# simongoricar/diploma_thesis-distributed_rendering_of_cgi_using_a_render_cluster

Measured on AMD Instinct MI355X. Metric: job frames/sec at 1/2/4/8 MI355X (04_very-simple); Mrays/s per GPU, higher is better.
Workload: dtype f32

## Files before the change

diploma_thesis-distributed_rendering_of_cgi_using_a_render_cluster_amd/csrc/paths.hpp:

```cpp
#pragma once

#include <hip/hip_runtime.h>

#include <algorithm>
#include <map>
#include <type_traits>
#include <utility>

#include "device.hpp"

namespace rr {

struct SceneArgs {
    const BvhNode* nodes;
    const QNode6* qnodes;
    const TriPack* tris;
    const float* mats;
    const float* lights;
    const float* filter;
    const float* mat_lut;
    int n_nodes, n_tris, n_mats, n_lights;
    int n_qnodes;
};

// ... 217 lines not shown
                const float3 wl = scl3(tl, rl);
                float3 b1, b2;
                make_onb(wl, b1, b2);
                float dx, dy;
                float u1, u2;
                rng2(key, dim0 + 1u, u1, u2);
                concentric_disk(u1, u2, dx, dy);
                dx = dx * radius;
                dy = dy * radius;
                const float3 sp = madd3(madd3(lp, b1, dx), b2, dy);
                const float3 ts = sub3(sp, P);
                const float ds2 = dot3(ts, ts);
                float id;
                sqrt_rcp_any(ds2, dist, id);
                wi = scl3(ts, id);
                const float cl = fabsf(dot3(wl, wi));
                Li = scl3(I, cl * id * id);
            } else {
                float id;
                sqrt_rcp_any(dl2, dist, id);
                wi = scl3(tl, id);
                Li = scl3(I, 1.0f / dl2);
            }
        } else {
            wi = mk3(-lt[4], -lt[5], -lt[6]);
            dist = kFltMax;
            Li = mk3(lt[8], lt[9], lt[10]);
        }
        const float cosN = dot3(N, wi);
        if (cosN > 0.0f) {
            float pdf;
            const float3 f = bsdf_eval_v(m, lut, vw, N, wo, wi, pdf);
            const float k = (float)fc.n_lights;
            float3 c = mk3(T.x * f.x * k * Li.x, T.y * f.y * k * Li.y, T.z * f.z * k * Li.z);
            if (bounce > 0) c = clamp_contrib(c, fc.clamp_indirect);
            if (max3f(c) > 0.0f) {
                out.shadow = true;
                if constexpr (Shadow::kInline) {
                    if (esc || !trace_shadow(Po, wi, dist)) add_to(L, c);
                } else {
                    out.so = Po;
                    out.sd = wi;
                    out.sdist = dist;
                    out.sc = c;
                }
            }
        }
    }
    float3 wi, f;
    float pdf;
    bool glossy;
    float u_b1, u_b2;
    rng2(key, dim0 + 4u, u_b1, u_b2);
    bool sampled;
    if constexpr (std::is_same<View, LdsView>::value) {
        const lds_f4w* fr = v.onb + kOnbF4 * h.idx + (flip ? 2 : 0);
        const float4 tb = lds_ld4(fr), bb = lds_ld4(fr + 1);
        sampled = bsdf_sample_onb(m, lut, vw, N, xyz(tb), mk3(tb.w, bb.x, bb.y), wo, u_lobe, u_b1, u_b2, wi, f, pdf,
                                  glossy);
    } else {
        sampled = bsdf_sample(m, lut, vw, N, wo, u_lobe, u_b1, u_b2, wi, f, pdf, glossy);
    }
    if (!sampled) return;
    const float k = 1.0f / pdf;
    T = mk3(T.x * f.x * k, T.y * f.y * k, T.z * f.z * k);
    if (!(max3f(T) > 0.0f)) return;
    if (bounce >= kRrStartBounce) {
        const float q = fminf(max3f(T), 1.0f);
        if (rng(key, dim0 + 6u) >= q) return;
        const float iq = 1.0f / q;
        T = mk3(T.x * iq, T.y * iq, T.z * iq);
    }
    out.cont = true;
    if constexpr (Cont::kInline) {
        on_cont(Po, wi, T, lob + (glossy ? kGlossyOne : 1u), esc, L);
        return;
    }
    out.o = Po;
    out.d = wi;
    out.T = T;
    out.lob = lob + (glossy ? kGlossyOne : 1u);
}

constexpr int kWavesPerBlock = kBlock / 64;
constexpr int kMaxBlocksPerCu = 8;

__device__ __forceinline__ void flush_counts(unsigned long long* __restrict__ tc, int slot, uint32_t nv,
                                             uint32_t nt) {
    unsigned long long a = nv, b = nt;
    for (int off = 32; off > 0; off >>= 1) {
        a += __shfl_xor(a, off);
        b += __shfl_xor(b, off);
    }
    if ((threadIdx.x & 63) == 0) {
        atomicAdd(&tc[slot], a);
        atomicAdd(&tc[slot + 1], b);
    }
}

RR_D void set_miss(Hit& h, float tmax) {
    h.t = tmax;
    h.u = h.v = 0.0f;
    h.idx = -1;
    h.orig = -1;
}

RR_D uchar4 tonemap(const FrameConsts& fc, float4 acc, const float* __restrict__ srgb) {
    float c[3] = {acc.x * fc.inv_spp * fc.exposure_scale, acc.y * fc.inv_spp * fc.exposure_scale,
                  acc.z * fc.inv_spp * fc.exposure_scale};
    uint8_t q[3];
    for (int k = 0; k < 3; ++k) {
        float v = fminf(fmaxf(c[k], 0.0f), 1.0f);
        if (fc.view_transform == 0) v = srgb_oetf(v, srgb, kSrgbN);
        q[k] = quantize8(v);
    }
    return make_uchar4(q[0], q[1], q[2], 255);
}

template <typename K>
int resident_grid(K kernel, size_t dyn_lds = 0, int block = kBlock) {
    int per_cu = 0;
    if (hipOccupancyMaxActiveBlocksPerMultiprocessor(&per_cu, kernel, block, dyn_lds) != hipSuccess || per_cu <= 0)
        per_cu = std::max(1, 1024 / block);
    return device_cu_count() * std::min(per_cu, kMaxBlocksPerCu * kBlock / block);
}
template <typename K>
int grid_for(K kernel, size_t dyn_lds, int block = kBlock) {
    static std::map<std::pair<const void*, size_t>, int> cache;
    const auto key = std::make_pair(reinterpret_cast<const void*>(kernel), dyn_lds);
    auto it = cache.find(key);
    if (it != cache.end()) return it->second;
    return cache[key] = resident_grid(kernel, dyn_lds, block);
}
inline int clamp_grid(long work, int resident, int block = kBlock) {
    const long g = (work + block - 1) / block;
    return (int)std::max<long>(1, std::min<long>(g, resident));
}

}
}
```

diploma_thesis-distributed_rendering_of_cgi_using_a_render_cluster_amd/csrc/rr_api.cpp:

```cpp
#include <hip/hip_runtime.h>

#include <cerrno>
#include <chrono>
#include <cmath>
#include <cstdlib>
#include <cstring>
#include <memory>
#include <string>
#include <unordered_set>
#include <vector>

#include "deflate.hpp"
#include "device.hpp"
#include "image_io.hpp"
#include "rr.h"
#include "scene.hpp"
#include "view.hpp"

using namespace rr;

static_assert(kMatLutIntervals == kMatLutN && kMatLutFloatsPerMat == kMatLutStride && kMatLutPsOffset == kMatLutPs,
              "scene.hpp material-table layout must match rr_device.h");

namespace {
// ... 1485 lines not shown
                    if (children) {
                        const uint32_t eb = (uint32_t)f2i(q.org.w);
                        for (int k = 0; k < kQWidth; ++k) {
                            const uint32_t lox = k < 4 ? (q.a.z >> (8 * k)) & 255u : (q.c.x >> (8 * (k - 4))) & 255u;
                            const uint32_t hix = k < 4 ? (q.b.y >> (8 * k)) & 255u : (q.c.y >> (16 + 8 * (k - 4))) & 255u;
                            const bool unused = lox == 255u && hix == 0u && !((eb >> (24 + k)) & 1u);
                            children[kQWidth * (size_t)i + k] = unused ? 0x7fffffff : q6_ref(q, k);
                        }
                    }
                    if (nodes16) std::memcpy(nodes16 + 16 * (size_t)i, &q, sizeof(QNode6));
                }
            }
            if (tri_orig) {
                std::vector<TriPack> tp((size_t)n);
                RR_HIP(hipMemcpyAsync(tp.data(), d.tris.ptr, (size_t)n * sizeof(TriPack), hipMemcpyDeviceToHost, st));
                RR_HIP(hipStreamSynchronize(st));
                for (int i = 0; i < n; ++i) tri_orig[i] = f2i(tp[(size_t)i].p0.w);
            }
        }
        return RR_OK;
    });
}

int rr_debug_trace(rr_ctx* c, rr_scene* s, int32_t frame, int32_t bvh_width, int32_t n, const float* rays,
                   float* hits, int32_t* prims, uint8_t* occluded) {
    if (!c || !s || n < 0 || (n > 0 && !rays)) return fail(RR_EINVAL, "bad arguments");
    if (bvh_width < 0 || bvh_width == 1 || bvh_width > 7)
        return fail(RR_EINVAL, "hierarchy must be 0 (frame's), 2 (LBVH), 3 (PLOC), 4 (6-wide), 5 (6-wide, packets) "
                               "6 (6-wide, one LDS stack entry) or 7 (6-wide, beam packets)");
    return guarded([&] {
        if (!idle(c)) return fail(RR_EBUSY, "submitted frames are pending");
        FrameSetup fs = setup_frame(s->desc, frame, nullptr);
        set_device(c);
        PinnedBuf staging;
        const int hier = bvh_width >= 5 ? kHierQWide : (bvh_width ? bvh_width : frame_hier_of(s, fs));
        prepare_frame(c, s, s->build, c->home, c->stream, fs, staging, hier);
        const int width = bvh_width >= 5 ? bvh_width : (hier == kHierQWide ? 4 : 2);
        hipStream_t st = c->stream;
        DevBuf<float4> dr, dh;
        DevBuf<int32_t> dp;
        DevBuf<uint8_t> dq;
        const size_t m = n > 0 ? (size_t)n : 1;
        dr.ensure(2 * m);
        dh.ensure(m);
        dp.ensure(m);
        dq.ensure(m);
        if (n > 0) RR_HIP(hipMemcpyAsync(dr.ptr, rays, (size_t)n * 8 * sizeof(float), hipMemcpyHostToDevice, st));
        trace_batch_device(s->mesh, s->build, c->paths, c->home, n, dr.ptr, dh.ptr, dp.ptr, dq.ptr, st, width);
        std::vector<float4> h(m);
        if (n > 0) {
            RR_HIP(hipMemcpyAsync(h.data(), dh.ptr, n * sizeof(float4), hipMemcpyDeviceToHost, st));
            if (prims) RR_HIP(hipMemcpyAsync(prims, dp.ptr, n * sizeof(int32_t), hipMemcpyDeviceToHost, st));
            if (occluded) RR_HIP(hipMemcpyAsync(occluded, dq.ptr, n, hipMemcpyDeviceToHost, st));
        }
        RR_HIP(hipStreamSynchronize(st));
        if (hits)
            for (int i = 0; i < n; ++i) {
                hits[4 * i] = h[i].x;
                hits[4 * i + 1] = h[i].y;
                hits[4 * i + 2] = h[i].z;
                hits[4 * i + 3] = 0.0f;
            }
        dr.release(); dh.release(); dp.release(); dq.release();
        return RR_OK;
    });
}

int rr_debug_tile_costs(rr_ctx* c, int32_t capacity, uint32_t* costs, int32_t* order, int32_t* n_tiles,
                        uint64_t* unit_log, int32_t unit_capacity) {
    if (!c || capacity < 0 || !n_tiles || (capacity > 0 && (!costs || !order)) || unit_capacity < 0 ||
        (unit_capacity > 0 && !unit_log))
        return fail(RR_EINVAL, "bad arguments");
    return guarded([&] {
        if (!idle(c)) return fail(RR_EBUSY, "submitted frames are pending");
        *n_tiles = 0;
        const FrameSlot* sl = c->last_enqueued;
        if (!sl || !sl->tiles) return RR_OK;
        set_device(c);
        const DevFrame& f = sl->dev;
        const size_t n = std::min(f.tile_cost.cap, f.tile_order.cap);
        *n_tiles = (int32_t)n;
        const size_t m = std::min<size_t>(n, (size_t)capacity);
        if (m > 0) {
            RR_HIP(hipMemcpy(costs, f.tile_cost.ptr, m * sizeof(uint32_t), hipMemcpyDeviceToHost));
            RR_HIP(hipMemcpy(order, f.tile_order.ptr, m * sizeof(int32_t), hipMemcpyDeviceToHost));
        }
        const size_t nu = std::min<size_t>((size_t)unit_capacity, kUnitLog);
        if (nu > 0) {
            std::memset(unit_log, 0, 2 * nu * sizeof(uint64_t));
            if (f.unit_logged && f.trav_counts.cap >= (size_t)(kTravWords + 2 * kUnitLog))
                RR_HIP(hipMemcpy(unit_log, f.trav_counts.ptr + kTravWords, 2 * nu * sizeof(uint64_t),
                                 hipMemcpyDeviceToHost));
        }
        return RR_OK;
    });
}

int rr_debug_fastmath_check(rr_ctx* c, uint32_t lo, uint64_t n, uint64_t* counts5) {
    if (!c || !counts5 || n > (1ull << 32) - lo) return fail(RR_EINVAL, "bad arguments");
    return guarded([&] {
        if (!idle(c)) return fail(RR_EBUSY, "submitted frames are pending");
        set_device(c);
        hipStream_t st = c->stream;
        DevBuf<unsigned long long> d;
        d.ensure(5);
        fastmath_check_device(lo, n, d.ptr, st);
        RR_HIP(hipMemcpyAsync(counts5, d.ptr, 5 * sizeof(uint64_t), hipMemcpyDeviceToHost, st));
        RR_HIP(hipStreamSynchronize(st));
        d.release();
        return RR_OK;
    });
}

int rr_debug_bsdf_sample(rr_ctx* c, const float* mat12, const float* n3, const float* wo3, int32_t n,
                         const float* u, float* wi3, float* f3, float* pdf, int32_t* ok) {
    if (!c || !mat12 || !n3 || !wo3 || n < 0 || (n > 0 && (!u || !wi3 || !f3 || !pdf || !ok)))
        return fail(RR_EINVAL, "bad arguments");
    return guarded([&] {
        if (!idle(c)) return fail(RR_EBUSY, "submitted frames are pending");
        set_device(c);
        hipStream_t st = c->stream;
        const size_t m = n > 0 ? (size_t)n : 1;
        DevBuf<float> dm, du, dw, df, dp, dl;
        DevBuf<int32_t> dk;
        float lut[kMatLutFloatsPerMat];
        build_material_lut(mat12, lut);
        dl.ensure(kMatLutFloatsPerMat);
        RR_HIP(hipMemcpyAsync(dl.ptr, lut, sizeof lut, hipMemcpyHostToDevice, st));
        dm.ensure(RR_MAT_FLOATS);
        du.ensure(3 * m); dw.ensure(3 * m); df.ensure(3 * m); dp.ensure(m); dk.ensure(m);
        RR_HIP(hipMemcpyAsync(dm.ptr, mat12, RR_MAT_FLOATS * sizeof(float), hipMemcpyHostToDevice, st));
        if (n > 0) RR_HIP(hipMemcpyAsync(du.ptr, u, 3 * (size_t)n * sizeof(float), hipMemcpyHostToDevice, st));
        bsdf_batch_device(dm.ptr, dl.ptr, n3, wo3, n, du.ptr, dw.ptr, df.ptr, dp.ptr, dk.ptr, st);
        if (n > 0) {
            RR_HIP(hipMemcpyAsync(wi3, dw.ptr, 3 * (size_t)n * sizeof(float), hipMemcpyDeviceToHost, st));
            RR_HIP(hipMemcpyAsync(f3, df.ptr, 3 * (size_t)n * sizeof(float), hipMemcpyDeviceToHost, st));
            RR_HIP(hipMemcpyAsync(pdf, dp.ptr, (size_t)n * sizeof(float), hipMemcpyDeviceToHost, st));
            RR_HIP(hipMemcpyAsync(ok, dk.ptr, (size_t)n * sizeof(int32_t), hipMemcpyDeviceToHost, st));
        }
        RR_HIP(hipStreamSynchronize(st));
        RR_HIP(hipStreamSynchronize(st));
        dm.release(); du.release(); dw.release(); df.release(); dp.release(); dk.release(); dl.release();
        return RR_OK;
    });
}

int rr_debug_object_matrix(rr_scene* s, int32_t obj, double frame, double* m16) {
    if (!s || !m16) return fail(RR_EINVAL, "NULL argument");
    return guarded([&] {
        object_matrix(s->desc, obj, frame, m16);
        return RR_OK;
    });
}

}
```

diploma_thesis-distributed_rendering_of_cgi_using_a_render_cluster_amd/csrc/tiles.hip:

```cpp
#pragma clang fp contract(off)

#include "paths.hpp"

#define RR_TILES_TU 1
#pragma clang diagnostic push
#pragma clang diagnostic ignored "-Wunused-function"
#include "wavefront.hip"
#pragma clang diagnostic pop

namespace rr {

namespace {

struct ShadeConsts {
    float3 world;
    float clamp_indirect;
    int max_bounces, max_diffuse, max_glossy, n_lights, n_tris;
};

RR_D void lds_copy(lds_f4w* dst, const float4* __restrict__ src, int n4) {
    const rr_f4v* s = reinterpret_cast<const rr_f4v*>(src);
    for (int i = threadIdx.x; i < n4; i += kBlock) dst[i] = s[i];
}
RR_D uint32_t hull_flags(lds_tri* tris, int n_tris, int i) {
// ... 135 lines not shown
        for (int i = threadIdx.x; i < a.n_tris; i += kBlock) {
            const TriPack tp = load_tri(v.tris, i);
            const float3 n = norm3(cross3(sub3(xyz(tp.p1), xyz(tp.p0)), sub3(xyz(tp.p2), xyz(tp.p0))));
            rr_f4v x;
            x.x = n.x; x.y = n.y; x.z = n.z;
            x.w = i2f(f2i(tp.p1.w) | (int)(hull_flags(v.tris, a.n_tris, i) << kHullShift));
            q[i] = x;
        }
        q += a.n_tris;
        v.matd = q;
        for (int i = threadIdx.x; i < a.n_mats; i += kBlock) {
            Mat m = load_mat(v.mats, i);
            mat_derive(m);
            rr_f4v r0, r1, r2, r3;
            r0.x = m.base.x; r0.y = m.base.y; r0.z = m.base.z; r0.w = m.roughness;
            r1.x = m.emission.x; r1.y = m.emission.y; r1.z = m.emission.z; r1.w = i2f(m.model);
            r2.x = m.alpha; r2.y = m.a2; r2.z = m.kd0; r2.w = i2f(m.spec_on);
            r3.x = m.cspec0.x; r3.y = m.cspec0.y; r3.z = m.cspec0.z; r3.w = 0.0f;
            q[kMatDF4 * i] = r0;
            q[kMatDF4 * i + 1] = r1;
            q[kMatDF4 * i + 2] = r2;
            q[kMatDF4 * i + 3] = r3;
        }
        q += kMatDF4 * a.n_mats;
        v.onb = q;
        __syncthreads();
        for (int j = threadIdx.x; j < 2 * a.n_tris; j += kBlock) {
            const int i = j >> 1, side = j & 1;
            const float4 nm = lds_ld4(v.nrm + i);
            const float3 n = side ? mk3(-nm.x, -nm.y, -nm.z) : xyz(nm);
            float3 t, b;
            make_onb(n, t, b);
            rr_f4v x, y;
            x.x = t.x; x.y = t.y; x.z = t.z; x.w = b.x;
            y.x = b.y; y.y = b.z; y.z = 0.0f; y.w = 0.0f;
            q[kOnbF4 * i + 2 * side] = x;
            q[kOnbF4 * i + 2 * side + 1] = y;
        }
        q += kOnbF4 * a.n_tris;
    }
    if constexpr (kCam) {
        v.cam = q;
        stage_camera(q, v.tris, a.n_tris, *cam_fc);
        q += kCamF4 * a.n_tris;
    }
    used = (int)(q - base);
    __syncthreads();
    return v;
}

template <bool kCount>
RR_D void camera_tris(const LdsView& v, uint64_t m0, uint64_t m1, const Shear& sh, int kz, float tmin, Hit& h,
                      TravCount& cnt) {
    for (int w = 0; w < 2; ++w) {
        uint64_t m = w ? m1 : m0;
        while (m) {
            const int i = (int)__builtin_ctzll(m) + 64 * w;
            m &= m - 1;
            if (kCount) ++cnt.tris;
            const lds_f4w* q = v.cam + kCamF4 * i + 3 * kz;
            const float4 ca = lds_ld4(q), cb = lds_ld4(q + 1), cc = lds_ld4(q + 2);
            float t, u, vv;
            if (woop_core(sh, xyz(ca), xyz(cb), xyz(cc), t, u, vv)) {
                const int orig = f2i(ca.w);
                if (closer(t, orig, tmin, h)) {
                    h.t = t;
                    h.u = u;
                    h.v = vv;
                    h.idx = i;
                    h.orig = orig;
                }
            }
        }
    }
}
template <bool kCount>
RR_D void camera_hit(const LdsView& v, uint64_t m0, uint64_t m1, float3 d, float tmin, float tmax, Hit& h,
                     TravCount& cnt) {
    set_miss(h, tmax);
    const Shear sh = make_shear_unit(d);
    camera_tris<kCount>(v, m0, m1, sh, sh.kz, tmin, h, cnt);
}

RR_D void tile_mask(const FrameConsts& fc, const LdsView& v, int n_tris, float x0, float x1, float y0, float y1,
                    uint64_t& m0, uint64_t& m1) {
    const float r = fc.filter_reach;
    const float X0 = x0 + 0.5f - r, X1 = x1 + 0.5f + r, Y0 = y0 + 0.5f - r, Y1 = y1 + 0.5f + r;
    const float Wf = (float)fc.W, Hf = (float)fc.H;
    constexpr float kEps = 0x1p-10f;
    uint64_t a = 0, b = 0;
    float best = 0.0f;
    for (int i = 0; i < n_tris; ++i) {
        const float4 q = lds_ld4(v.cam + kCamF4 * i + kCamRect);
        bool in = !(q.y < X0 || q.x > X1 || q.w < Y0 || q.z > Y1);
        bool cov = true;
        float pl[3] = {0.0f, 0.0f, 0.0f};
        for (int k = 0; k < 3 && in; ++k) {
            const float4 l = lds_ld4(v.cam + kCamF4 * i + kCamRect + 1 + k);
            const float m = l.x * (l.x > 0.0f ? X1 : X0) + l.y * (l.y > 0.0f ? Y1 : Y0) + l.z;
            in = m >= -1.0f;
            cov = cov && l.x * (l.x > 0.0f ? X0 : X1) + l.y * (l.y > 0.0f ? Y0 : Y1) + l.z >= 1.0f;
            pl[k] = l.w;
        }
        if (in) {
            if (i < 64) a |= 1ull << i;
            else b |= 1ull << (i - 64);
            if (cov) {
                const float e = kEps * (fabsf(pl[0]) * Wf + fabsf(pl[1]) * Hf + fabsf(pl[2]));
                const float lo = pl[0] * (pl[0] > 0.0f ? X0 : X1) + pl[1] * (pl[1] > 0.0f ? Y0 : Y1) + pl[2] - e;
                const float hi = pl[0] * (pl[0] > 0.0f ? X1 : X0) + pl[1] * (pl[1] > 0.0f ? Y1 : Y0) + pl[2] + e;
                if (lo > 0.0f && hi * fc.clip_start * (1.0f + kEps) < 1.0f && lo * fc.clip_end > 1.0f + kEps)
                    best = fmaxf(best, lo);
            }
        }
    }
    if (best > 0.0f) {
        for (int i = 0; i < n_tris; ++i) {
            const lds_f4w* l = v.cam + kCamF4 * i + kCamRect + 1;
            const float pa = lds_ld4(l).w, pb = lds_ld4(l + 1).w, pc = lds_ld4(l + 2).w;
            const float e = kEps * (fabsf(pa) * Wf + fabsf(pb) * Hf + fabsf(pc));
            const float lo = pa * (pa > 0.0f ? X0 : X1) + pb * (pb > 0.0f ? Y0 : Y1) + pc - e;
            const float hi = pa * (pa > 0.0f ? X1 : X0) + pb * (pb > 0.0f ? Y1 : Y0) + pc + e;
            if (lo > 0.0f && hi < best) {
                if (i < 64) a &= ~(1ull << i);
                else b &= ~(1ull << (i - 64));
            }
        }
    }
    m0 = ((uint64_t)(uint32_t)__builtin_amdgcn_readfirstlane((int)(uint32_t)(a >> 32)) << 32) |
         (uint32_t)__builtin_amdgcn_readfirstlane((int)(uint32_t)a);
    m1 = ((uint64_t)(uint32_t)__builtin_amdgcn_readfirstlane((int)(uint32_t)(b >> 32)) << 32) |
         (uint32_t)__builtin_amdgcn_readfirstlane((int)(uint32_t)b);
}

constexpr int kTile = 8;
#ifndef RR_TILE_SHARDS
#define RR_TILE_SHARDS 8
#endif
constexpr int kTileShards = RR_TILE_SHARDS;
constexpr int kTileCtrStride = 32;

struct TileOrder {
    int tx, n;
    int bx0, by0, bw, bh;
    RR_D void at(int i, int& x, int& y) const {
        const int nb = bw * bh;
        if (i < nb) {
            y = i / bw;
            x = bx0 + (i - y * bw);
            y += by0;
            return;
        }
        int j = i - nb;
        const int ntop = by0 * tx;
        if (j < ntop) {
            y = j / tx;
            x = j - y * tx;
            return;
        }
        j -= ntop;
        const int rw = tx - bw, nmid = bh * rw;
        if (j < nmid) {
            const int r = j / rw, cx = j - r * rw;
            y = by0 + r;
            x = cx < bx0 ? cx : cx + bw;
            return;
        }
        j -= nmid;
        y = j / tx;
        x = j - y * tx;
        y += by0 + bh;
    }
};

RR_D TileOrder tile_order(const FrameConsts& fc, const ScreenCull& sc) {
    TileOrder to;
    to.tx = (fc.W + kTile - 1) / kTile;
    const int ty = (fc.H + kTile - 1) / kTile;
    to.n = to.tx * ty;
    to.bx0 = to.by0 = 0;
    to.bw = to.tx;
    to.bh = ty;
    if (!sc.on) return to;
    const float m = fc.filter_reach + 1.0f;
    const float x0 = fmaxf(sc.r[0] - m, 0.0f), x1 = fminf(sc.r[1] + m, (float)fc.W - 1.0f);
    const float y0 = fmaxf(sc.r[2] - m, 0.0f), y1 = fminf(sc.r[3] + m, (float)fc.H - 1.0f);
    if (!(x0 <= x1 && y0 <= y1)) {
        to.bw = to.bh = 0;
        return to;
    }
    to.bx0 = (int)x0 / kTile;
    to.by0 = (int)y0 / kTile;
    to.bw = (int)x1 / kTile - to.bx0 + 1;
    to.bh = (int)y1 / kTile - to.by0 + 1;
    return to;
}

RR_D bool tile_culled(const FrameConsts& fc, const ScreenCull& sc, int tx, int ty) {
    if (!sc.on) return false;
    const float x0 = (float)(tx * kTile) + 0.5f, y0 = (float)(ty * kTile) + 0.5f;
    const float x1 = x0 + (float)(kTile - 1), y1 = y0 + (float)(kTile - 1);
    const float r = fc.filter_reach;
    return x1 + r < sc.r[0] || x0 - r > sc.r[1] || y1 + r < sc.r[2] || y0 - r > sc.r[3];
}

RR_D int uniform_i(int x) { return __builtin_amdgcn_readfirstlane(x); }
RR_D float uniform_f(float x) { return __int_as_float(__builtin_amdgcn_readfirstlane(__float_as_int(x))); }
RR_D ScreenCull uniform_cull(ScreenCull c) {
    c.on = uniform_i(c.on ? 1 : 0) != 0;
    for (int k = 0; k < 4; ++k) c.r[k] = uniform_f(c.r[k]);
    return c;
}
RR_D TileOrder uniform_order(TileOrder t) {
    t.tx = uniform_i(t.tx);
    t.n = uniform_i(t.n);
// ... 118 lines not shown
            add_to(L, clamp_contrib(mul3(T, sc.world), sc.clamp_indirect));
        else
            L = tiles_continue<kCount>(sc, v, o, d, T, lob, key, L, tt);
    }
};

}
struct TileSlices {
    int n;
    size_t floats;
    float* slab;
    const int32_t* order;
    uint32_t* cost;
};
namespace {

template <bool kCount, bool kWhole>
RR_D void tiles_body(const FrameConsts& fc, const LdsView& v, uint32_t* __restrict__ tile_ctr, float4* __restrict__ film,
                     const float* __restrict__ srgb, uchar4* __restrict__ out, uint32_t* __restrict__ tot,
                     int32_t* __restrict__ spill, unsigned long long* __restrict__ tc, lds_int* stack,
                     const TileSlices sl, unsigned long long rt_entry, lds_uint* cont_ctr) {
    const int stride = gridDim.x * kBlock;
    unsigned long long clk0 = 0, rt0 = 0;
    if (kCount) {
        clk0 = __builtin_amdgcn_s_memtime();
        rt0 = __builtin_amdgcn_s_memrealtime();
    }
    const TileTrav tt{stack, spill, stride, tot + drops_slot(fc.max_bounces), cont_ctr + kWctr * (threadIdx.x >> 6), tc};
    TravCount cp;
    uint32_t n_c0 = 0, n_s0 = 0, n_c1 = 0, n_s1 = 0, n_t0 = 0;
    const ScreenCull cull = uniform_cull(screen_cull(fc, v.nodes));
    const TileOrder to = uniform_order(tile_order(fc, cull));
    const int lane = threadIdx.x & 63;
    const int ng = (fc.spp_total + kFilmGroup - 1) / kFilmGroup;
    const int nb = to.bw * to.bh;
    const int n_slices = kWhole ? 1 : sl.n;
    const int n_sliced = nb * n_slices;
    const int n_units = n_sliced + (to.n - nb);
    const int n_shards = min((int)gridDim.x, kTileShards);
    const int shard = (int)blockIdx.x % n_shards;
    float4 bg = make_float4(0.0f, 0.0f, 0.0f, 0.0f);
    for (int g = 0; g < ng; ++g) {
        float3 P = mk3(0.0f, 0.0f, 0.0f);
        const int s_end = min(fc.spp_total, (g + 1) * kFilmGroup);
        for (int s = g * kFilmGroup; s < s_end; ++s) add_to(P, fc.world);
        bg.x = bg.x + P.x;
        bg.y = bg.y + P.y;
        bg.z = bg.z + P.z;
    }
    bg = make_float4(uniform_f(bg.x), uniform_f(bg.y), uniform_f(bg.z), 0.0f);
    const uchar4 bg_px = __builtin_bit_cast(uchar4, uniform_i(__builtin_bit_cast(int, tonemap(fc, bg, srgb))));
    for (;;) {
        int t, k = 0, nk = 1;
        int u = 0;
        if (lane == 0) u = (int)atomicAdd(tile_ctr + shard * kTileCtrStride, 1u);
        u = __builtin_amdgcn_readlane(u, 0) * n_shards + shard;
        if (u >= n_units) break;
        if (u < n_sliced) {
            const int j = kWhole ? u : u / n_slices;
            k = kWhole ? 0 : u - j * n_slices;
            nk = n_slices;
            t = uniform_i(sl.order[j]);
        } else {
            t = nb + (u - n_sliced);
        }
        const unsigned long long u_start = __builtin_amdgcn_s_memrealtime();
        int tx, ty;
        to.at(t, tx, ty);
        const int px = tx * kTile + (lane & (kTile - 1)), py = ty * kTile + (lane >> 3);
        const bool valid = px < fc.W && py < fc.H;
        const int pix = py * fc.W + px;
        float4 acc = make_float4(0.0f, 0.0f, 0.0f, 0.0f);
        if (tile_culled(fc, cull, tx, ty)) {
            if (k != 0) continue;
            if (valid) {
                film[pix] = bg;
                out[pix] = bg_px;
            }
            continue;
        }
        const int s_lo = nk > 1 ? k * kFilmGroup : 0;
        const int s_hi = nk > 1 ? min(fc.spp_total, s_lo + kFilmGroup) : fc.spp_total;
        uint64_t cm0, cm1;
        tile_mask(fc, v, fc.n_tris, (float)(tx * kTile), (float)(tx * kTile + kTile - 1), (float)(ty * kTile),
                  (float)(ty * kTile + kTile - 1), cm0, cm1);
        const uint32_t pk = pixel_key(fc.seed, (uint32_t)pix);
        const int s_run = (cm0 | cm1) != 0 ? s_hi : s_lo;
        float3 P = mk3(0.0f, 0.0f, 0.0f);
        auto group_end = [&](int s) {
            if ((s + 1) % kFilmGroup == 0 || s + 1 == s_hi) {
                acc.x = acc.x + P.x;
                acc.y = acc.y + P.y;
                acc.z = acc.z + P.z;
                P = mk3(0.0f, 0.0f, 0.0f);
            }
        };
        for (int s = s_run; s < s_hi; ++s) {
            add_to(P, fc.world);
            group_end(s);
        }
        for (int s = s_lo; s < s_run; ++s) {
            const uint32_t key = sample_key(pk, (uint32_t)s);
            float3 o = mk3(0.0f, 0.0f, 0.0f), d = o, L = o;
            float tmin = 0.0f, tmax = -1.0f;
            bool culled = true;
            if (valid) camera_ray_xy(fc, v.filter, px, py, key, o, d, tmin, tmax, &cull, &culled);
            n_t0 += wave_count(!culled);
            bool cont = false, shadow = false;
            if (valid) {
                Hit h;
                set_miss(h, tmax);
                if (!culled) camera_hit<kCount>(v, cm0, cm1, d, tmin, tmax, h, cp);
                ShadeOut so;
                const ShadeConsts sc{fc.world, fc.clamp_indirect, fc.max_bounces, fc.max_diffuse, fc.max_glossy,
                                     fc.n_lights, fc.n_tris};
                if constexpr ((RR_TILES_CONT_INPLACE & (kWhole ? 1 : 2)) != 0) {
                    shade(fc, 0, v, o, d, mk3(1.0f, 1.0f, 1.0f), 0u, h, key, L, so,
                          InlineShadow<kCount>{v, fc.n_tris, tt}, TileCont<kCount>{sc, v, tt, key});
                } else {
                    shade(fc, 0, v, o, d, mk3(1.0f, 1.0f, 1.0f), 0u, h, key, L, so,
                          InlineShadow<kCount>{v, fc.n_tris, tt});
                    if (so.cont) TileCont<kCount>{sc, v, tt, key}(so.o, so.d, so.T, so.lob, so.esc, L);
                }
                cont = so.cont;
                shadow = so.shadow;
            }
            n_c0 += wave_count(cont);
            n_s0 += wave_count(shadow);
            add_to(P, L);
            group_end(s);
        }
        if (!kWhole && nk > 1) {
            float* const slab = sl.slab + (size_t)t * sl.floats + (size_t)k * 192;
            slab[lane] = acc.x;
            slab[64 + lane] = acc.y;
            slab[128 + lane] = acc.z;
        } else if (valid) {
            film[pix] = acc;
            out[pix] = tonemap(fc, acc, srgb);
        }
        if (lane == 0) {
            const unsigned long long u_end = __builtin_amdgcn_s_memrealtime();
            atomicAdd(&sl.cost[ty * to.tx + tx], (uint32_t)(u_end - u_start));
            if ((kCount || RR_TILES_LOG_ALWAYS) && u < kUnitLog) {
                tc[kTravWords + 2 * u] = u_start;
                tc[kTravWords + 2 * u + 1] = u_end;
            }
        }
    }
    uint32_t* const tail = tot + camera_traced_slot(fc.max_bounces);
    n_c1 = tt.wctr[0];
    n_s1 = tt.wctr[1];
    flush_rays(tot, n_c0, n_s0, n_c1, n_s1, tail, n_t0, tt.wctr[2], tt.wctr[3]);
    if (kCount && lane == 0) {
        atomicAdd(&tc[2], (unsigned long long)tt.wctr[4]);
        atomicAdd(&tc[3], (unsigned long long)tt.wctr[5]);
        atomicAdd(&tc[4], (unsigned long long)tt.wctr[6]);
        atomicAdd(&tc[5], (unsigned long long)tt.wctr[7]);
    }
    if (kCount) {
        flush_counts(tc, 0, cp.nodes, cp.tris);
        const unsigned long long clk1 = __builtin_amdgcn_s_memtime(), rt1 = __builtin_amdgcn_s_memrealtime();
        if ((threadIdx.x & 63) == 0) {
            atomicAdd(&tc[6], clk1 - clk0);
            atomicAdd(&tc[7], rt1 - rt0);
            atomicAdd(&tc[8], 1ull);
            atomicAdd(&tc[9], rt1 - rt_entry);
            atomicMax(&tc[10], ~rt_entry);
            atomicMax(&tc[11], rt1);
            atomicMax(&tc[12], rt_entry);
            atomicMax(&tc[13], ~rt1);
        }
    }
}

#ifndef RR_TILES_WAVES
#define RR_TILES_WAVES 4
#endif
#ifndef RR_TILES_WAVES_WHOLE
#define RR_TILES_WAVES_WHOLE 5
#endif
template <bool kCount, bool kWhole>
__global__ __launch_bounds__(kBlock, kWhole ? RR_TILES_WAVES_WHOLE : RR_TILES_WAVES) void k_tiles(FrameConsts fc,
                                                                                                 SceneArgs sa,
// ... 83 lines not shown
        }
        const int pix = py * fc.W + px;
        film[pix] = acc;
        out[pix] = tonemap(fc, acc, srgb);
    }
}

int film_groups(int spp) { return (spp + kFilmGroup - 1) / kFilmGroup; }
size_t tile_slab_bytes(int spp, long tiles) {
    const int ng = film_groups(spp);
    return ng > 1 ? (size_t)192 * sizeof(float) * ng * (size_t)tiles : 0;
}
constexpr size_t kTileSlabMax = (size_t)16 << 30;
size_t scene_lds_bytes(const FrameConsts& fc, bool shading) {
    const int n_nodes = std::max(fc.n_tris - 1, 1);
    size_t f4 = 4 * (size_t)n_nodes + kTriF4 * (size_t)fc.n_tris;
    if (shading)
        f4 += (3 + kMatDF4 + kMatLutStride / 4) * (size_t)fc.n_mats + 3 * (size_t)fc.n_lights + kFilterN / 4 +
              (size_t)(1 + kOnbF4) * fc.n_tris;
    return 16 * f4;
}
}

constexpr size_t kTilesStaticLds = sizeof(int) * (size_t)(kLdsStack * kBlock + kWctr * kWavesPerBlock);
size_t tiles_dyn_lds_bytes(const FrameConsts& fc) {
    return scene_lds_bytes(fc, true) + 16 * (size_t)kCamF4 * (size_t)fc.n_tris;
}
constexpr int kTilesMinBlocks = 3;
constexpr size_t kCuLds = 160 * 1024;
bool scene_in_lds(int n_tris, int n_mats, int n_lights) {
    FrameConsts fc{};
    fc.n_tris = n_tris;
    fc.n_mats = n_mats;
    fc.n_lights = n_lights;
    return n_tris > 0 && n_tris <= 128 &&
           kTilesMinBlocks * (kTilesStaticLds + tiles_dyn_lds_bytes(fc)) <= kCuLds;
}

bool frame_uses_tiles(const FrameConsts& base, bool force_wavefront) {
    const long n_tiles = (long)((base.W + 7) / 8) * ((base.H + 7) / 8);
    return scene_in_lds(base.n_tris, base.n_mats, base.n_lights) && !force_wavefront &&
           tile_slab_bytes(base.spp_total, n_tiles) <= kTileSlabMax;
}

namespace {
struct TileGrid {
    decltype(&k_tiles<false, false>) kx;
    size_t dyn;
    int grid;
    TileGrid(const FrameConsts& fc, bool count, bool whole) {
        dyn = tiles_dyn_lds_bytes(fc);
        kx = count ? (whole ? k_tiles<true, true> : k_tiles<true, false>)
                   : (whole ? k_tiles<false, true> : k_tiles<false, false>);
        grid = grid_for(kx, dyn);
    }
};
}

void render_tiles_device(const DevMesh& m, DevBuild& s, DevPaths& p, DevFrame& f, const FrameConsts& base, int n_chunks,
                         FrameOpts o, hipStream_t st) {
    const int npix = base.npix;
    const TileGrid G(base, o.count_traversal, o.tile_whole);
    if (p.grid_blocks == 0) p.grid_blocks = device_cu_count() * kMaxBlocksPerCu;
    f.ensure_spill(p.grid_blocks);
    f.film.ensure((size_t)npix);
    f.rgba8.ensure((size_t)npix * 4);
    const int cpc = counters_per_chunk(base.max_bounces);
    const long tiles = (long)((base.W + 7) / 8) * ((base.H + 7) / 8);
    const size_t n_ctr = (size_t)cpc * n_chunks;
    f.counters.ensure(n_ctr);
    unsigned long long* tc = nullptr;
    if (o.count_traversal || RR_TILES_LOG_ALWAYS) {
        f.trav_counts.ensure(kTravWords + 2 * kUnitLog);
        RR_HIP(hipMemsetAsync(f.trav_counts.ptr, 0, (kTravWords + 2 * kUnitLog) * sizeof(unsigned long long), st));
        tc = f.trav_counts.ptr;
        f.unit_logged = true;
    }
    const SceneArgs sa{s.nodes.ptr, s.qnodes.ptr, s.tris.ptr, f.materials.ptr, f.lights.ptr, p.filter_table.ptr,
                       f.mat_lut.ptr, std::max(m.n_tris - 1, 1), m.n_tris, base.n_mats, base.n_lights, s.nq};
    FrameConsts fc = base;
    fc.first_sample = 0;
    fc.spp_chunk = base.spp_total;
    uint32_t* tot = reinterpret_cast<uint32_t*>(f.counters.ptr);
    if (f.tile_cost.cap < (size_t)tiles) {
        f.tile_cost.ensure((size_t)tiles);
        RR_HIP(hipMemsetAsync(f.tile_cost.ptr, 0, sizeof(uint32_t) * tiles, st));
    }
    f.tile_order.ensure((size_t)tiles);
    TileSlices sl{o.tile_whole ? 1 : film_groups(base.spp_total), (size_t)192 * film_groups(base.spp_total), nullptr,
                  f.tile_order.ptr, f.tile_cost.ptr};
    f.tile_slices = sl.n;
    if (sl.n > 1) {
        f.tile_slab.ensure(sl.floats * (size_t)tiles);
        sl.slab = f.tile_slab.ptr;
    }
    const int g = clamp_grid(tiles * 64, G.grid);
    f.prof.begin(st, RR_K_TILES);
    f.tile_ctrs.ensure((size_t)kTileShards * kTileCtrStride);
    k_tile_order<<<1, kOrderThreads, 0, st>>>(fc, s.nodes.ptr, f.tile_cost.ptr, f.tile_order.ptr, f.tile_ctrs.ptr,
                                              reinterpret_cast<uint32_t*>(f.counters.ptr), (int)n_ctr);
    G.kx<<<g, kBlock, G.dyn, st>>>(fc, sa, f.tile_ctrs.ptr, f.film.ptr, p.srgb_lut.ptr,
                                           reinterpret_cast<uchar4*>(f.rgba8.ptr), tot, f.spill.ptr, tc, sl);
    if (sl.n > 1)
        k_tiles_fold<<<(int)std::min<long>((tiles + kWavesPerBlock - 1) / kWavesPerBlock, 2048), kBlock, 0, st>>>(
            fc, s.nodes.ptr, sl, f.film.ptr, p.srgb_lut.ptr, reinterpret_cast<uchar4*>(f.rgba8.ptr));
    f.prof.end(st);
    RR_HIP(hipGetLastError());
}

}
```

diploma_thesis-distributed_rendering_of_cgi_using_a_render_cluster_amd/native.py:

```python
from __future__ import annotations

import ctypes
import os
from dataclasses import dataclass

import numpy as np

_HERE = os.path.dirname(os.path.abspath(__file__))
LIB_PATH = os.path.join(_HERE, "lib", "librr.so")
SHIM_PATH = os.path.join(_HERE, "lib", "rr-blender-shim")

RR_OK, RR_ENOENT, RR_EIO, RR_ENOMEM, RR_ENODEV, RR_EINVAL, RR_ENOTSUP = 0, -2, -5, -12, -19, -22, -95
RR_EBUSY = -16
RR_MAX_FRAMES_IN_FLIGHT = 3
RR_VIEW_SCENE, RR_VIEW_STANDARD, RR_VIEW_RAW, RR_VIEW_FILMIC = -1, 0, 1, 2
RR_VIEW_FILMIC_LOG, RR_VIEW_FALSE_COLOR = 3, 4
LOOKS = ["None", "Very High Contrast", "High Contrast", "Medium High Contrast", "Medium Contrast",
         "Medium Low Contrast", "Low Contrast", "Very Low Contrast"]
RR_ABI_VERSION = 8
QWIDTH = 6
RR_CAM_FLOATS, RR_LIGHT_FLOATS, RR_MAT_FLOATS, RR_RENDER_INTS, RR_RENDER_FLOATS = 16, 12, 12, 10, 4


class RRError(RuntimeError):
# ... 438 lines not shown
        if n.value > out.size:
            raise RRError(RR_EINVAL, f"device PNG of {n.value} bytes exceeds the {out.size}-byte buffer")
        return out[:n.value].tobytes()

    def exr_device(self, rgba: np.ndarray) -> bytes:
        rgba = np.ascontiguousarray(rgba, dtype=np.float32)
        h, w = rgba.shape[:2]
        out = np.zeros(8 * w * h + 16 * ((h + 15) // 16) + 1024, np.uint8)
        n = ctypes.c_uint64()
        _check(lib().rr_debug_exr_device(self.handle, _ptr(rgba, ctypes.c_float), w, h,
                                         _ptr(out, ctypes.c_uint8), out.size, ctypes.byref(n)), self.handle)
        if n.value > out.size:
            raise RRError(RR_EINVAL, f"device EXR of {n.value} bytes exceeds the {out.size}-byte buffer")
        return out[:n.value].tobytes()

    def set_exr_depth(self, depth: int = 0):
        _check(lib().rr_set_exr_depth(self.handle, int(depth)), self.handle)

    def set_color_mode(self, mode=0):
        _check(lib().rr_set_color_mode(self.handle, color_mode_value(mode)), self.handle)

    def set_look(self, name: str | None = None):
        _check(lib().rr_set_look(self.handle, name.encode() if name else None), self.handle)

    def set_display_gamma(self, gamma: float = 0.0):
        _check(lib().rr_set_display_gamma(self.handle, ctypes.c_float(gamma)), self.handle)

    def set_dither(self, intensity=0.0):
        v = RR_DITHER_SCENE if intensity == "scene" else float(intensity)
        _check(lib().rr_set_dither(self.handle, ctypes.c_float(v)), self.handle)

    def view_device(self, rgba: np.ndarray, view_transform: int = 0, exposure_scale: float = 1.0) -> np.ndarray:
        rgba = np.ascontiguousarray(rgba, dtype=np.float32)
        h, w = rgba.shape[:2]
        out = np.zeros((h, w, 4), np.uint8)
        _check(lib().rr_debug_view_device(self.handle, _ptr(rgba, ctypes.c_float), w, h, int(view_transform),
                                          ctypes.c_float(exposure_scale), _ptr(out, ctypes.c_uint8)), self.handle)
        return out

    def encode_device(self, fmt: str, image: np.ndarray, depth: int = 0, color_mode=0, view_transform: int = 0,
                      exposure_scale: float = 1.0, quality: int = 90) -> bytes:
        is_float = image.dtype != np.uint8
        image = np.ascontiguousarray(image, dtype=np.float32 if is_float else np.uint8)
        h, w = image.shape[:2]
        args = (self.handle, fmt.encode(), int(depth), color_mode_value(color_mode),
                image.ctypes.data_as(ctypes.c_void_p), 1 if is_float else 0, w, h, int(view_transform),
                ctypes.c_float(exposure_scale), int(quality))
        n = ctypes.c_uint64()
        _check(lib().rr_debug_encode_device(*args, None, 0, ctypes.byref(n)), self.handle)
        out = np.zeros(n.value, np.uint8)
        _check(lib().rr_debug_encode_device(*args, _ptr(out, ctypes.c_uint8), out.size, ctypes.byref(n)), self.handle)
        if n.value > out.size:
            raise RRError(RR_EINVAL, f"device file of {n.value} bytes exceeds the {out.size}-byte buffer")
        return out[:n.value].tobytes()

    def exr32_device(self, rgba: np.ndarray) -> bytes:
        rgba = np.ascontiguousarray(rgba, dtype=np.float32)
        h, w = rgba.shape[:2]
        out = np.zeros(16 * w * h + 16 * ((h + 15) // 16) + 1024, np.uint8)
        n = ctypes.c_uint64()
        _check(lib().rr_debug_exr32_device(self.handle, _ptr(rgba, ctypes.c_float), w, h,
                                           _ptr(out, ctypes.c_uint8), out.size, ctypes.byref(n)), self.handle)
        if n.value > out.size:
            raise RRError(RR_EINVAL, f"device EXR of {n.value} bytes exceeds the {out.size}-byte buffer")
        return out[:n.value].tobytes()

    def bsdf_sample(self, mat12, n, wo, u):
        f32 = lambda a: np.ascontiguousarray(a, dtype=np.float32)
        m, n, wo, u = f32(mat12), f32(n), f32(wo), f32(u).reshape(-1, 3)
        k = u.shape[0]
        wi, f = np.zeros((k, 3), np.float32), np.zeros((k, 3), np.float32)
        pdf, ok = np.zeros(k, np.float32), np.zeros(k, np.int32)
        _check(lib().rr_debug_bsdf_sample(self.handle, _ptr(m, ctypes.c_float), _ptr(n, ctypes.c_float),
                                          _ptr(wo, ctypes.c_float), k, _ptr(u, ctypes.c_float),
                                          _ptr(wi, ctypes.c_float), _ptr(f, ctypes.c_float),
                                          _ptr(pdf, ctypes.c_float), _ptr(ok, ctypes.c_int32)), self.handle)
        return wi, f, pdf, ok

    def fastmath_check(self, lo: int = 0, n: int = 1 << 32):
        out = (ctypes.c_uint64 * 5)()
        _check(lib().rr_debug_fastmath_check(self.handle, int(lo), int(n), out), self.handle)
        return tuple(int(v) for v in out)

    def tile_costs(self, capacity: int = 1 << 20, units: int = 1 << 16):
        costs = np.zeros(capacity, np.uint32)
        order = np.zeros(capacity, np.int32)
        log = np.zeros((max(units, 1), 2), np.uint64)
        n = ctypes.c_int32(0)
        _check(lib().rr_debug_tile_costs(self.handle, capacity, _ptr(costs, ctypes.c_uint32),
                                         _ptr(order, ctypes.c_int32), ctypes.byref(n),
                                         _ptr(log, ctypes.c_uint64), units), self.handle)
        m = min(int(n.value), capacity)
        return costs[:m], order[:m], log[:units]

    def trace(self, scene: Scene, frame: int, rays: np.ndarray, width: int = 0):
        rays = np.ascontiguousarray(rays, dtype=np.float32).reshape(-1, 8)
        n = rays.shape[0]
        hits = np.zeros((max(n, 1), 4), np.float32)
        prims = np.zeros(max(n, 1), np.int32)
        occ = np.zeros(max(n, 1), np.uint8)
        _check(lib().rr_debug_trace(self.handle, scene.handle, int(frame), int(width), n, _ptr(rays, ctypes.c_float),
                                    _ptr(hits, ctypes.c_float), _ptr(prims, ctypes.c_int32),
                                    _ptr(occ, ctypes.c_uint8)), self.handle)
        return hits[:n], prims[:n], occ[:n]


def srgb16_table() -> np.ndarray:
    n = ctypes.c_int32()
    _check(lib().rr_debug_srgb16_table(None, 0, ctypes.byref(n)))
    t = np.zeros(n.value, np.float32)
    _check(lib().rr_debug_srgb16_table(_ptr(t, ctypes.c_float), t.size, ctypes.byref(n)))
    return t


def display_gamma(values: np.ndarray, gamma: float) -> np.ndarray:
    v = np.ascontiguousarray(values, dtype=np.float32)
    out = np.zeros_like(v)
    _check(lib().rr_debug_display_gamma(_ptr(v.reshape(-1), ctypes.c_float), v.size, ctypes.c_float(gamma),
                                        _ptr(out.reshape(-1), ctypes.c_float)))
    return out


def sin_fixed(values: np.ndarray) -> np.ndarray:
    v = np.ascontiguousarray(values, dtype=np.float32)
    out = np.zeros_like(v)
    _check(lib().rr_debug_sin_fixed(_ptr(v.reshape(-1), ctypes.c_float), v.size, _ptr(out.reshape(-1), ctypes.c_float)))
    return out


def dither_noise(width: int, height: int) -> np.ndarray:
    out = np.zeros((int(height), int(width)), np.float32)
    _check(lib().rr_debug_dither_noise(int(width), int(height), _ptr(out.reshape(-1), ctypes.c_float)))
    return out


def encode_image(rgba: np.ndarray, out_path_no_ext: str, fmt: str, quality: int = 90) -> int:
    rgba = np.ascontiguousarray(rgba, dtype=np.uint8)
    h, w = rgba.shape[:2]
    nbytes = ctypes.c_uint64()
    _check(lib().rr_encode_image(_ptr(rgba, ctypes.c_uint8), w, h, out_path_no_ext.encode(), fmt.encode(),
                                 int(quality), ctypes.byref(nbytes)))
    return nbytes.value


def encode_image_mode(rgba: np.ndarray, out_path_no_ext: str, fmt: str, quality: int = 90, color_mode=0) -> int:
    rgba = np.ascontiguousarray(rgba, dtype=np.uint8)
    h, w = rgba.shape[:2]
    nbytes = ctypes.c_uint64()
    _check(lib().rr_encode_image_mode(_ptr(rgba, ctypes.c_uint8), w, h, out_path_no_ext.encode(), fmt.encode(),
                                      int(quality), color_mode_value(color_mode), ctypes.byref(nbytes)))
    return nbytes.value
```

Measured before the change: 1205.

## Add fast path for tiles fully covered by a single triangle

When the tile mask finds exactly one triangle that covers the whole tile, and that triangle is also the nearest-depth cover, the tile kernel now intersects camera rays against that one triangle only. It shades through a specialised shade_covered routine instead of the generic camera-hit path. This avoids per-sample mask iteration and generic material lookups for simple scenes. It adds per-tile cost logging in a doubled tile_cost buffer and some register pressure from the extra code path.

```diff
diff --git a/diploma_thesis-distributed_rendering_of_cgi_using_a_render_cluster_amd/csrc/paths.hpp b/diploma_thesis-distributed_rendering_of_cgi_using_a_render_cluster_amd/csrc/paths.hpp
--- a/diploma_thesis-distributed_rendering_of_cgi_using_a_render_cluster_amd/csrc/paths.hpp
+++ b/diploma_thesis-distributed_rendering_of_cgi_using_a_render_cluster_amd/csrc/paths.hpp
@@ -323,6 +323,162 @@
     out.lob = lob + (glossy ? kGlossyOne : 1u);
 }
 
+struct CoveredInLoop {
+    static constexpr bool kHeld = false;
+};
+struct CoveredHeld {
+    static constexpr bool kHeld = true;
+    float3 N;
+    int mid;
+    bool esc;
+    Mat m;
+    float3 tb, bb;
+    float lt[11];
+};
+template <typename Shadow, typename FC, typename Cont, typename Held = CoveredInLoop>
+__device__ __forceinline__ void shade_covered(const FC& fc, int bounce, const LdsView& v, int tri, bool flip, bool hit,
+                                              float3 o, float3 d, float3 T, uint32_t lob, const Hit& h, uint32_t key,
+                                              float3& L, ShadeOut& out, const Shadow& trace_shadow,
+                                              const Cont& on_cont, const Held& held = Held{}) {
+    static_assert(Shadow::kInline, "the shadow ray is traced in place");
+    out.cont = false;
+    out.shadow = false;
+    out.esc = false;
+    if (!hit) {
+        float3 c = mul3(T, fc.world);
+        if (bounce > 0) c = clamp_contrib(c, fc.clamp_indirect);
+        add_to(L, c);
+        return;
+    }
+    float3 N;
+    int mid;
+    bool esc;
+    Mat m;
+    if constexpr (Held::kHeld) {
+        N = held.N;
+        mid = held.mid;
+        esc = held.esc;
+        m = held.m;
+    } else {
+        const float4 nm = lds_ld4(v.nrm + tri);
+        N = xyz(nm);
+        mid = f2i(nm.w) & ((1 << kHullShift) - 1);
+        const uint32_t hull = (uint32_t)f2i(nm.w) >> kHullShift;
+        m = view_mat(v, mid);
+        if (flip) N = mk3(-N.x, -N.y, -N.z);
+        esc = ((hull >> (flip ? 1 : 0)) & 1u) != 0u;
+    }
+    __builtin_assume(mid >= 0 && mid < 4096);
+    const auto lut = v.lut + kMatLutStride * mid;
+    const float t = h.t;
+    const float3 P = madd3(o, d, t);
+    out.esc = esc;
+    const float3 wo = mk3(-d.x, -d.y, -d.z);
+    if (m.emission.x != 0.0f || m.emission.y != 0.0f || m.emission.z != 0.0f) {
+        float3 c = mul3(T, m.emission);
+        if (bounce > 0) c = clamp_contrib(c, fc.clamp_indirect);
+        add_to(L, c);
+    }
+    if (path_capped(fc, bounce, lob)) return;
+    const BsdfView vw = bsdf_view(m, lut, N, wo);
+    const uint32_t dim0 = 2u + (uint32_t)(kDimsPerBounce * bounce);
+    float u_light, u_lobe;
+    rng2(key, dim0, u_light, u_lobe);
+    const float3 Po = offset_ray(P, N);
+    if (fc.n_lights > 0) {
+        const auto lt = [&](int k) {
+            if constexpr (Held::kHeld) return held.lt[k];
+            else return v.lights[k];
+        };
+        float3 wi, Li;
+        float dist;
+        if (lt(0) == 0.0f) {
+            const float3 lp = mk3(lt(1), lt(2), lt(3));
+            const float radius = lt(7);
+            const float3 I = mk3(lt(8), lt(9), lt(10));
+            const float3 tl = sub3(lp, P);
+            const float dl2 = dot3(tl, tl);
+            if (radius > 0.0f) {
+                float sl, rl;
+                sqrt_rcp_any(dl2, sl, rl);
+                const float3 wl = scl3(tl, rl);
+                float3 b1, b2;
+                make_onb(wl, b1, b2);
+                float dx, dy;
+                float u1, u2;
+                rng2(key, dim0 + 1u, u1, u2);
+                concentric_disk(u1, u2, dx, dy);
+                dx = dx * radius;
+                dy = dy * radius;
+                const float3 sp = madd3(madd3(lp, b1, dx), b2, dy);
+                const float3 ts = sub3(sp, P);
+                const float ds2 = dot3(ts, ts);
+                float id;
+                sqrt_rcp_any(ds2, dist, id);
+                wi = scl3(ts, id);
+                const float cl = fabsf(dot3(wl, wi));
+                Li = scl3(I, cl * id * id);
+            } else {
+                float id;
+                sqrt_rcp_any(dl2, dist, id);
+                wi = scl3(tl, id);
+                Li = scl3(I, 1.0f / dl2);
+            }
+        } else {
+            wi = mk3(-lt(4), -lt(5), -lt(6));
+            dist = kFltMax;
+            Li = mk3(lt(8), lt(9), lt(10));
+        }
+        const float cosN = dot3(N, wi);
+        if (cosN > 0.0f) {
+            float pdf;
+            const float3 f = bsdf_eval_v(m, lut, vw, N, wo, wi, pdf);
+            const float k = (float)fc.n_lights;
+            float3 c = mk3(T.x * f.x * k * Li.x, T.y * f.y * k * Li.y, T.z * f.z * k * Li.z);
+            if (bounce > 0) c = clamp_contrib(c, fc.clamp_indirect);
+            if (max3f(c) > 0.0f) {
+                out.shadow = true;
+                if (esc || !trace_shadow(Po, wi, dist)) add_to(L, c);
+            }
+        }
+    }
+    float3 wi, f;
+    float pdf;
+    bool glossy;
+    float u_b1, u_b2;
+    rng2(key, dim0 + 4u, u_b1, u_b2);
+    float3 ft, fb;
+    if constexpr (Held::kHeld) {
+        ft = held.tb;
+        fb = held.bb;
+    } else {
+        const lds_f4w* fr = v.onb + kOnbF4 * tri + (flip ? 2 : 0);
+        const float4 tb = lds_ld4(fr), bb = lds_ld4(fr + 1);
+        ft = xyz(tb);
+        fb = mk3(tb.w, bb.x, bb.y);
+    }
+    if (!bsdf_sample_onb(m, lut, vw, N, ft, fb, wo, u_lobe, u_b1, u_b2, wi, f, pdf, glossy))
+        return;
+    const float k = 1.0f / pdf;
+    T = mk3(T.x * f.x * k, T.y * f.y * k, T.z * f.z * k);
+    if (!(max3f(T) > 0.0f)) return;
+    if (bounce >= kRrStartBounce) {
+        const float q = fminf(max3f(T), 1.0f);
+        if (rng(key, dim0 + 6u) >= q) return;
+        const float iq = 1.0f / q;
+        T = mk3(T.x * iq, T.y * iq, T.z * iq);
+    }
+    out.cont = true;
+    if constexpr (Cont::kInline) {
+        on_cont(Po, wi, T, lob + (glossy ? kGlossyOne : 1u), esc, L);
+        return;
+    }
+    out.o = Po;
+    out.d = wi;
+    out.T = T;
+    out.lob = lob + (glossy ? kGlossyOne : 1u);
+}
+
 constexpr int kWavesPerBlock = kBlock / 64;
 constexpr int kMaxBlocksPerCu = 8;
 
diff --git a/diploma_thesis-distributed_rendering_of_cgi_using_a_render_cluster_amd/csrc/rr_api.cpp b/diploma_thesis-distributed_rendering_of_cgi_using_a_render_cluster_amd/csrc/rr_api.cpp
--- a/diploma_thesis-distributed_rendering_of_cgi_using_a_render_cluster_amd/csrc/rr_api.cpp
+++ b/diploma_thesis-distributed_rendering_of_cgi_using_a_render_cluster_amd/csrc/rr_api.cpp
@@ -1591,7 +1591,8 @@
         *n_tiles = (int32_t)n;
         const size_t m = std::min<size_t>(n, (size_t)capacity);
         if (m > 0) {
-            RR_HIP(hipMemcpy(costs, f.tile_cost.ptr, m * sizeof(uint32_t), hipMemcpyDeviceToHost));
+            const size_t mc = std::min<size_t>(f.tile_cost.cap, (size_t)capacity);
+            RR_HIP(hipMemcpy(costs, f.tile_cost.ptr, mc * sizeof(uint32_t), hipMemcpyDeviceToHost));
             RR_HIP(hipMemcpy(order, f.tile_order.ptr, m * sizeof(int32_t), hipMemcpyDeviceToHost));
         }
         const size_t nu = std::min<size_t>((size_t)unit_capacity, kUnitLog);
diff --git a/diploma_thesis-distributed_rendering_of_cgi_using_a_render_cluster_amd/csrc/tiles.hip b/diploma_thesis-distributed_rendering_of_cgi_using_a_render_cluster_amd/csrc/tiles.hip
--- a/diploma_thesis-distributed_rendering_of_cgi_using_a_render_cluster_amd/csrc/tiles.hip
+++ b/diploma_thesis-distributed_rendering_of_cgi_using_a_render_cluster_amd/csrc/tiles.hip
@@ -241,14 +241,18 @@
     camera_tris<kCount>(v, m0, m1, sh, sh.kz, tmin, h, cnt);
 }
 
+#ifndef RR_TILES_COVERED
+#define RR_TILES_COVERED 1
+#endif
 RR_D void tile_mask(const FrameConsts& fc, const LdsView& v, int n_tris, float x0, float x1, float y0, float y1,
-                    uint64_t& m0, uint64_t& m1) {
+                    uint64_t& m0, uint64_t& m1, int& covered) {
     const float r = fc.filter_reach;
     const float X0 = x0 + 0.5f - r, X1 = x1 + 0.5f + r, Y0 = y0 + 0.5f - r, Y1 = y1 + 0.5f + r;
     const float Wf = (float)fc.W, Hf = (float)fc.H;
     constexpr float kEps = 0x1p-10f;
     uint64_t a = 0, b = 0;
     float best = 0.0f;
+    int best_i = -1;
     for (int i = 0; i < n_tris; ++i) {
         const float4 q = lds_ld4(v.cam + kCamF4 * i + kCamRect);
         bool in = !(q.y < X0 || q.x > X1 || q.w < Y0 || q.z > Y1);
@@ -268,8 +272,10 @@
                 const float e = kEps * (fabsf(pl[0]) * Wf + fabsf(pl[1]) * Hf + fabsf(pl[2]));
                 const float lo = pl[0] * (pl[0] > 0.0f ? X0 : X1) + pl[1] * (pl[1] > 0.0f ? Y0 : Y1) + pl[2] - e;
                 const float hi = pl[0] * (pl[0] > 0.0f ? X1 : X0) + pl[1] * (pl[1] > 0.0f ? Y1 : Y0) + pl[2] + e;
-                if (lo > 0.0f && hi * fc.clip_start * (1.0f + kEps) < 1.0f && lo * fc.clip_end > 1.0f + kEps)
+                if (lo > 0.0f && hi * fc.clip_start * (1.0f + kEps) < 1.0f && lo * fc.clip_end > 1.0f + kEps) {
+                    if (lo > best) best_i = i;
                     best = fmaxf(best, lo);
+                }
             }
         }
     }
@@ -290,6 +296,11 @@
          (uint32_t)__builtin_amdgcn_readfirstlane((int)(uint32_t)a);
     m1 = ((uint64_t)(uint32_t)__builtin_amdgcn_readfirstlane((int)(uint32_t)(b >> 32)) << 32) |
          (uint32_t)__builtin_amdgcn_readfirstlane((int)(uint32_t)b);
+    covered = -1;
+    if (RR_TILES_COVERED && best_i >= 0 && __popcll(m0) + __popcll(m1) == 1) {
+        const int only = m0 ? (int)__builtin_ctzll(m0) : 64 + (int)__builtin_ctzll(m1);
+        covered = only == __builtin_amdgcn_readfirstlane(best_i) ? only : -1;
+    }
 }
 
 constexpr int kTile = 8;
@@ -574,8 +585,9 @@
         const int s_lo = nk > 1 ? k * kFilmGroup : 0;
         const int s_hi = nk > 1 ? min(fc.spp_total, s_lo + kFilmGroup) : fc.spp_total;
         uint64_t cm0, cm1;
+        int cov;
         tile_mask(fc, v, fc.n_tris, (float)(tx * kTile), (float)(tx * kTile + kTile - 1), (float)(ty * kTile),
-                  (float)(ty * kTile + kTile - 1), cm0, cm1);
+                  (float)(ty * kTile + kTile - 1), cm0, cm1, cov);
         const uint32_t pk = pixel_key(fc.seed, (uint32_t)pix);
         const int s_run = (cm0 | cm1) != 0 ? s_hi : s_lo;
         float3 P = mk3(0.0f, 0.0f, 0.0f);
@@ -591,7 +603,80 @@
             add_to(P, fc.world);
             group_end(s);
         }
-        for (int s = s_lo; s < s_run; ++s) {
+        bool covered = cov >= 0 && tx * kTile + kTile <= fc.W && ty * kTile + kTile <= fc.H && fc.n_lights <= 1;
+        if (covered && cull.on) {
+            const float r = fc.filter_reach, cx = (float)(tx * kTile) + 0.5f, cy = (float)(ty * kTile) + 0.5f;
+            covered = cx - r >= cull.r[0] && cx + (float)(kTile - 1) + r <= cull.r[1] && cy - r >= cull.r[2] &&
+                      cy + (float)(kTile - 1) + r <= cull.r[3];
+        }
+        int s_gen = s_run;
+        if (RR_TILES_COVERED && covered) {
+            const float4 nm = lds_ld4(v.nrm + cov), a0 = lds_ld4(v.cam + kCamF4 * cov);
+            const bool flip = uniform_i(dot3(xyz(nm), mk3(a0.z, a0.x, a0.y)) > 0.0f ? 1 : 0) != 0;
+#if RR_TILES_COVERED == 2
+            CoveredHeld held;
+            {
+                const auto uf3 = [](float3 a) { return mk3(uniform_f(a.x), uniform_f(a.y), uniform_f(a.z)); };
+                const int word = uniform_i(f2i(nm.w));
+                held.mid = word & ((1 << kHullShift) - 1);
+                held.esc = ((((uint32_t)word >> kHullShift) >> (flip ? 1 : 0)) & 1u) != 0u;
+                held.N = uf3(flip ? mk3(-nm.x, -nm.y, -nm.z) : xyz(nm));
+                const Mat m = view_mat(v, held.mid);
+                held.m.base = uf3(m.base);
+                held.m.roughness = uniform_f(m.roughness);
+                held.m.emission = uf3(m.emission);
+                held.m.model = uniform_i(m.model);
+                held.m.alpha = uniform_f(m.alpha);
+                held.m.a2 = uniform_f(m.a2);
+                held.m.kd0 = uniform_f(m.kd0);
+                held.m.spec_on = uniform_i(m.spec_on);
+                held.m.cspec0 = uf3(m.cspec0);
+                held.m.metallic = held.m.specular = held.m.ior = 0.0f;
+                const lds_f4w* fr = v.onb + kOnbF4 * cov + (flip ? 2 : 0);
+                const float4 tb = lds_ld4(fr), bb = lds_ld4(fr + 1);
+                held.tb = uf3(xyz(tb));
+                held.bb = uf3(mk3(tb.w, bb.x, bb.y));
+                for (int k = 0; k < 11; ++k) held.lt[k] = fc.n_lights > 0 ? uniform_f(v.lights[k]) : 0.0f;
+            }
+#else
+            const CoveredInLoop held;
+#endif
+            for (int s = s_lo; s < s_hi; ++s) {
+                const uint32_t key = sample_key(pk, (uint32_t)s);
+                float3 o, d, L = mk3(0.0f, 0.0f, 0.0f);
+                float tmin, tmax;
+                camera_ray_xy(fc, v.filter, px, py, key, o, d, tmin, tmax);
+                n_t0 += 64u;
+                const Shear sh = make_shear_unit(d);
+                if (kCount) ++cp.tris;
+                const lds_f4w* q = v.cam + kCamF4 * cov + 3 * sh.kz;
+                const float4 ca = lds_ld4(q), cb = lds_ld4(q + 1), cc = lds_ld4(q + 2);
+                Hit h;
+                set_miss(h, tmax);
+                float t = tmax, u, vv;
+                bool hit = woop_core(sh, xyz(ca), xyz(cb), xyz(cc), t, u, vv);
+                hit = hit && closer(t, f2i(ca.w), tmin, h);
+                h.t = hit ? t : tmax;
+                ShadeOut so;
+                const ShadeConsts sc{fc.world, fc.clamp_indirect, fc.max_bounces, fc.max_diffuse, fc.max_glossy,
+                                     fc.n_lights, fc.n_tris};
+                if constexpr ((RR_TILES_CONT_INPLACE & (kWhole ? 1 : 2)) != 0) {
+                    shade_covered(fc, 0, v, cov, flip, hit, o, d, mk3(1.0f, 1.0f, 1.0f), 0u, h, key, L, so,
+                                  InlineShadow<kCount>{v, fc.n_tris, tt}, TileCont<kCount>{sc, v, tt, key}, held);
+                } else {
+                    shade_covered(fc, 0, v, cov, flip, hit, o, d, mk3(1.0f, 1.0f, 1.0f), 0u, h, key, L, so,
+                                  InlineShadow<kCount>{v, fc.n_tris, tt}, EmitCont{}, held);
+                    if (so.cont) TileCont<kCount>{sc, v, tt, key}(so.o, so.d, so.T, so.lob, so.esc, L);
+                }
+                n_c0 += wave_count(so.cont);
+                n_s0 += wave_count(so.shadow);
+                add_to(P, L);
+                group_end(s);
+            }
+            s_gen = s_lo;
+            if (kCount && lane == 0) atomicAdd(&sl.cost[to.n + ty * to.tx + tx], (uint32_t)(s_hi - s_lo));
+        }
+        for (int s = s_lo; s < s_gen; ++s) {
             const uint32_t key = sample_key(pk, (uint32_t)s);
             float3 o = mk3(0.0f, 0.0f, 0.0f), d = o, L = o;
             float tmin = 0.0f, tmax = -1.0f;
@@ -841,10 +926,12 @@
     fc.first_sample = 0;
     fc.spp_chunk = base.spp_total;
     uint32_t* tot = reinterpret_cast<uint32_t*>(f.counters.ptr);
-    if (f.tile_cost.cap < (size_t)tiles) {
-        f.tile_cost.ensure((size_t)tiles);
+    if (f.tile_cost.cap < 2 * (size_t)tiles) {
+        f.tile_cost.ensure(2 * (size_t)tiles);
         RR_HIP(hipMemsetAsync(f.tile_cost.ptr, 0, sizeof(uint32_t) * tiles, st));
     }
+    if (o.count_traversal)
+        RR_HIP(hipMemsetAsync(f.tile_cost.ptr + tiles, 0, sizeof(uint32_t) * tiles, st));
     f.tile_order.ensure((size_t)tiles);
     TileSlices sl{o.tile_whole ? 1 : film_groups(base.spp_total), (size_t)192 * film_groups(base.spp_total), nullptr,
                   f.tile_order.ptr, f.tile_cost.ptr};
diff --git a/diploma_thesis-distributed_rendering_of_cgi_using_a_render_cluster_amd/native.py b/diploma_thesis-distributed_rendering_of_cgi_using_a_render_cluster_amd/native.py
--- a/diploma_thesis-distributed_rendering_of_cgi_using_a_render_cluster_amd/native.py
+++ b/diploma_thesis-distributed_rendering_of_cgi_using_a_render_cluster_amd/native.py
@@ -544,7 +544,7 @@
         _check(lib().rr_debug_fastmath_check(self.handle, int(lo), int(n), out), self.handle)
         return tuple(int(v) for v in out)
 
-    def tile_costs(self, capacity: int = 1 << 20, units: int = 1 << 16):
+    def tile_costs(self, capacity: int = 1 << 20, units: int = 1 << 16, raw: bool = False):
         costs = np.zeros(capacity, np.uint32)
         order = np.zeros(capacity, np.int32)
         log = np.zeros((max(units, 1), 2), np.uint64)
@@ -553,7 +553,7 @@
                                          _ptr(order, ctypes.c_int32), ctypes.byref(n),
                                          _ptr(log, ctypes.c_uint64), units), self.handle)
         m = min(int(n.value), capacity)
-        return costs[:m], order[:m], log[:units]
+        return (costs if raw else costs[:m]), order[:m], log[:units]
 
     def trace(self, scene: Scene, frame: int, rays: np.ndarray, width: int = 0):
         rays = np.ascontiguousarray(rays, dtype=np.float32).reshape(-1, 8)
```

Measured after the change: 1290, median of 6. 7.1% higher.
